# jtdaugherty/flux

Measured on AMD Instinct MI355X. Metric: Msamples/sec on demo2.yml (fixed spp), higher is better.
Workload: dtype f64

## Files before the change

flux_amd/build.py:

```python
import os
import shutil
import subprocess
import sys

ROOT = os.path.dirname(os.path.dirname(os.path.abspath(__file__)))
CSRC = os.path.join(ROOT, "flux_amd", "csrc")
HIP_SOURCES = ["abi.hip", "multi.hip", "tables.hip", "render.hip", "bvh.cpp", "scene_build.cpp", "launch_plan.cpp"]
HIP_HEADERS = ["flux_ctx.h", "scene_build.h", "joining_thread.h", "flux_device.h", "flux_plan.h", "flux_rng.h", "flux_tables.h", "flux_bvh.h", "flux_math.h",
               "flux_math_coeffs.h", "flux_env_verdict.h", "render_body.inc"]
HIP_LIB = os.path.join(ROOT, "flux_amd", "libflux_hip.so")

HIP_FLAGS = ["--offload-arch=gfx950", "-O3", "-std=c++17", "-fPIC", "-shared", "-ffp-contract=off",
             "-fno-fast-math", "-Wall", "-Wno-unused-function",
             "-mllvm", "-disable-machine-licm"]


def _newer(target, deps):
    if not os.path.exists(target):
        return True
    t = os.path.getmtime(target)
    return any(os.path.getmtime(d) > t for d in deps)


def _hipcc():
    for cand in (os.environ.get("HIPCC"), shutil.which("hipcc"), "/opt/rocm/bin/hipcc"):
        if cand and os.path.exists(cand):
            return cand
    raise RuntimeError("hipcc not found (set HIPCC)")


KERNEL_FILES = ["render.hip", "render_body.inc", "tables.hip", "flux_device.h", "flux_plan.h", "flux_bvh.h", "flux_math.h",
                "flux_math_coeffs.h", "flux_rng.h", "flux_tables.h", "flux_env_verdict.h"]


def build_id(extra_flags=()):
    import hashlib

    def digest(names):
        h = hashlib.sha256()
        h.update(" ".join(HIP_FLAGS + list(extra_flags)).encode())
        for n in names:
            path = os.path.join(ROOT, "include", n) if n == "flux_abi.h" else os.path.join(CSRC, n)
            h.update(n.encode() + b"\0")
            with open(path, "rb") as f:
                h.update(f.read())
        return h.hexdigest()[:16]
    return f"lib:{digest(sorted(set(HIP_SOURCES + HIP_HEADERS + ['flux_abi.h'])))} kernels:{digest(KERNEL_FILES)}"


def _id_flag(extra_flags=()):
    return "-DFLUX_BUILD_ID=\"" + build_id(extra_flags) + "\""


def build_variant(out_path, extra_flags, verbose=False):
    srcs = [os.path.join(CSRC, s) for s in HIP_SOURCES]
    flags = [f for f in HIP_FLAGS if not (f == "-ffp-contract=off" and any(x.startswith("-ffp-contract") for x in extra_flags))]
    cmd = [_hipcc()] + flags + list(extra_flags) + [_id_flag(extra_flags), "-o", out_path] + srcs
    if verbose:
        print(" ".join(cmd), file=sys.stderr)
    subprocess.run(cmd, check=True, cwd=CSRC)
    return out_path


def build_hip(force=False, verbose=False):
    srcs = [os.path.join(CSRC, s) for s in HIP_SOURCES]
# ... 38 lines not shown
```

flux_amd/csrc/abi.hip:

```cpp
#include <hip/hip_runtime.h>

#include <chrono>
#include <cmath>
#include <cstdarg>
#include <cstdio>
#include <cstring>
#include <memory>
#include <new>
#include <algorithm>
#include <cstdlib>
#include <string>
#include <vector>

#include "../../include/flux_abi.h"
#include "flux_device.h"
#include "flux_tables.h"
#include "flux_math_coeffs.h"

#include "flux_ctx.h"

namespace flux {

thread_local std::string g_last_error;

// ... 491 lines not shown
    p.first_row = 0;
    p.row_stride = 1;
    p.num_rows = (int32_t)ctx->H;
    p.set_first = (int32_t)first_set;
    p.set_stride = (int32_t)set_stride;
    p.set_count = (int32_t)num_sets;
    p.out_by_set = 1;
    p.slot_first = (int32_t)((first_set - ctx->sets.first) / ctx->sets.stride);
    p.slot_stride = (int32_t)(set_stride / ctx->sets.stride);
    return apply_traversal(ctx, p);
}

int flux_ctx_launch_plan(flux_ctx *ctx, uint64_t num_rows, uint64_t num_sets, int64_t out[FLUX_PLAN_WORDS]) {
    if (!ctx || !out) return fail(FLUX_E_INVALID, "null argument");
    if (num_rows > ctx->H) return fail(FLUX_E_INVALID, "%llu rows exceed image height %u", (unsigned long long)num_rows, ctx->H);
    flux::RenderParams p;
    if (num_sets == 0) {
        p = rows_params(ctx, 0, 1, num_rows, nullptr);
    } else {
        const uint64_t held = ctx->sets.count;
        if (num_sets > held) return fail(FLUX_E_INVALID, "%llu sets exceed the %llu this context holds", (unsigned long long)num_sets,
                                         (unsigned long long)held);
        p = sets_params(ctx, ctx->sets.first, ctx->sets.stride, num_sets, nullptr);
    }
    const flux::LaunchPlan L = flux::plan_render(p, ctx->variant, effective_math(ctx));
    out[0] = L.kernel;
    out[1] = L.block;
    out[2] = (int64_t)L.blocks;
    out[3] = (int64_t)L.lds;
    out[4] = L.waves_per_pixel;
    out[5] = effective_math(ctx);
    out[6] = (ctx->math == FLUX_MATH_FAST && ctx->rp.glossy_long) ? (strict_fits_lds(ctx) ? FLUX_ROUTE_TO_STRICT : FLUX_ROUTE_KEPT_FAST)
                                                                 : FLUX_ROUTE_NONE;
    out[7] = 0;
    return FLUX_OK;
}

int flux_render_rows_device(flux_ctx *ctx, uint64_t first_row, uint64_t row_stride, uint64_t num_rows,
                            void *d_out_rgb, void *hip_stream) {
    if (!ctx) return fail(FLUX_E_INVALID, "null context");
    if (num_rows == 0) return FLUX_OK;
    if (!d_out_rgb) return fail(FLUX_E_INVALID, "null output pointer");
    if (row_stride < 1) return fail(FLUX_E_INVALID, "row_stride must be >= 1");
    if (!holds_all_sets(ctx))
        return fail(FLUX_E_INVALID, "rendering rows needs all sample sets; this context holds the share %u + k*%u "
                    "(flux_ctx_create_sets): use flux_render_sets_device", ctx->sets.first, ctx->sets.stride);
    if (first_row >= ctx->H || first_row + (num_rows - 1) * row_stride >= ctx->H)
        return fail(FLUX_E_INVALID, "rows %llu + k*%llu (k<%llu) exceed image height %u",
                    (unsigned long long)first_row, (unsigned long long)row_stride,
                    (unsigned long long)num_rows, ctx->H);
    DeviceGuard guard(ctx->device);
    if (!guard.ok) return fail(FLUX_E_DEVICE, "hipSetDevice(%d) failed", ctx->device);
    hipStream_t stream = (hipStream_t)hip_stream;
    const flux::RenderParams p = rows_params(ctx, first_row, row_stride, num_rows, (double *)d_out_rgb);
    if (int rc = check_lds_budget(ctx, p, "flux_render_rows")) return rc;
    HIP_TRY(hipEventRecord(ctx->ev0, stream));
    HIP_TRY(flux::launch_render(p, ctx->variant, effective_math(ctx), stream));
    HIP_TRY(hipEventRecord(ctx->ev1, stream));
    ctx->timed = true;
    return FLUX_OK;
}

int flux_render_sets_device(flux_ctx *ctx, uint64_t first_set, uint64_t set_stride, uint64_t num_sets, void *d_out_rgb,
                            void *hip_stream) {
    if (!ctx) return fail(FLUX_E_INVALID, "null context");
    if (num_sets == 0) return FLUX_OK;
    if (!d_out_rgb) return fail(FLUX_E_INVALID, "null output pointer");
// ... 205 lines not shown
```

flux_amd/csrc/flux_device.h:

```cpp
#pragma once
#include <hip/hip_runtime.h>
#include <stdint.h>

#include "flux_bvh.h"
#include "flux_env_verdict.h"


#ifndef FLUX_UNI_SPHERES
#define FLUX_UNI_SPHERES 2
#endif
#ifndef FLUX_BVH_WIDE_MAX_STACK
#define FLUX_BVH_WIDE_MAX_STACK 48
#endif
#ifndef FLUX_MAX_WAVES_PER_PIXEL
#define FLUX_MAX_WAVES_PER_PIXEL 4
#endif
#ifndef FLUX_MIN_SAMPLES_PER_WAVE
#define FLUX_MIN_SAMPLES_PER_WAVE 4096
#endif

namespace flux {

constexpr int kHemiDoubles = 4;
constexpr double kTMin = 0.0005;
constexpr double kPi = 3.14159265358979323846264338327950288;
constexpr double kInvPi = 1.0 / kPi;

constexpr int kShapeSphere = 0;
constexpr int kShapePlane = 1;
constexpr int kShapeDisk = 2;
constexpr int kShapeBox = 3;
constexpr int kMatMatte = 0;
constexpr int kMatEmissive = 1;
constexpr int kMatReflective = 2;
constexpr int kMatGlossy = 3;
constexpr int kMatDielectric = 4;

struct DevShape {
// ... 157 lines not shown
```

flux_amd/csrc/flux_plan.h:

```cpp
#pragma once
#include <stddef.h>
#include <stdint.h>

#include "flux_device.h"

#ifndef FLUX_BLOCK_THREADS
#define FLUX_BLOCK_THREADS 64
#endif
#ifndef FLUX_WPE_SPLIT
#define FLUX_WPE_SPLIT 5
#endif
#ifndef FLUX_HITQ_MIN_TAKE
#define FLUX_HITQ_MIN_TAKE 32
#endif

namespace flux {

constexpr int kGlossExpSlots = 4;

constexpr int kQueueDoubles = 9;
constexpr int kQueueBytesPerWave = (kQueueDoubles * 64) * 8 + 2 * 64 * 4;
constexpr int kHitQDoubles = 7;
constexpr int kHitQInts = 3;
constexpr int kHitQBytesPerSlot = kHitQDoubles * 8 + kHitQInts * 4;
enum HitQField : uint32_t {
    kHitQOx = 0, kHitQOy = 2, kHitQOz = 4, kHitQDx = 6, kHitQDy = 8, kHitQDz = 10, kHitQT = 12,
    kHitQHitDepth = 14,
    kHitQSample = 15,
    kHitQList = 16,
};
constexpr uint32_t kHitQDwordsPerSlot = kHitQBytesPerSlot / 4;
constexpr uint32_t hitq_entry_dword(uint32_t C, uint32_t k) { return (C - 1u - k) * kHitQDwordsPerSlot; }
constexpr bool hitq_admits_phase_a(uint32_t C, uint32_t nhit) { return nhit + 64u <= C; }

constexpr size_t kTputEntryBytes = 24;
constexpr size_t kTputTableMaxBytes = (size_t)4 << 20;
constexpr uint32_t tput_index(uint32_t list_bits, uint32_t ml) { return (1u << list_bits) | ml; }
size_t tput_table_bytes(const RenderParams &p, int *bits = nullptr);

enum KernelCopy { kCopyStrict = 0, kCopyFast = 1, kCopyFastDiel = 2 };
KernelCopy kernel_copy(const RenderParams &p, int math);

struct LaunchPlan {
    int kernel = -1;
    unsigned block = 64;
    uint64_t blocks = 0;
    size_t lds = 0;
    unsigned waves_per_pixel = 1;
    int lds_scene = 0;
    int hq_cap = 0, hq_th = 0, hq_bits = 0;
    int copy = kCopyFast;
    int tris = 0;
    int typ = 0;
    int max32 = 0;
    int uniform_a = 1;
};
LaunchPlan plan_render(const RenderParams &p, int variant, int math);

size_t lane_stacks_lds(int math, size_t depth, bool tris, size_t bvh_stack, size_t lanes);
size_t shade_rays_lds(const RenderParams &p, int math);

}
```

flux_amd/csrc/launch_plan.cpp:

```cpp
#include <algorithm>
#include <cstdlib>

#include "flux_plan.h"
#include "../../include/flux_abi.h"

namespace flux {

KernelCopy kernel_copy(const RenderParams &p, int math) {
    if (math == FLUX_MATH_STRICT) return kCopyStrict;
    return p.has_diel ? kCopyFastDiel : kCopyFast;
}

size_t lane_stacks_lds(int math, size_t depth, bool tris, size_t bvh_stack, size_t lanes) {
    return (math == FLUX_MATH_STRICT ? depth * 4 * lanes * sizeof(double) : 0) + (tris ? bvh_stack * lanes * sizeof(int) : 0);
}

size_t shade_rays_lds(const RenderParams &p, int math) {
    return lane_stacks_lds(math, (size_t)p.max_depth, p.n_tris > 0, (size_t)p.bvh_stack, 64);
}

static bool split_typ(const RenderParams &p) {
    return p.n_sph <= 32 && p.glossy_long == 0 && p.unit_dirs == 1 && p.self_skip == 1 && p.env_short == 1 && p.n_uni == 1 &&
           p.fsph32 != nullptr && p.n_dsk == 0 && p.n_box == 0 && p.has_diel == 0 && (p.n_gloss_exp == 0 || p.gx_stride != 0);
}
// ... 65 lines not shown
        L.block = 64;
        size_t lds4 = (size_t)(p.bvh4_stack > 0 ? p.bvh4_stack : 1) * 64 * sizeof(int);
        const size_t scene4 = (size_t)hit_records(p) * sizeof(DevHitRec) + (size_t)p.n_mats * sizeof(DevMaterial) +
                              (size_t)p.n_sph * sizeof(DevScanSphere);
        const bool lds_scene4 = lds4 + scene4 <= 7680;
        if (lds_scene4) lds4 += scene4;
        if (p.nodes4 != nullptr && p.bvh4_stack <= FLUX_BVH_WIDE_MAX_STACK) {
            L.kernel = 4;
            L.lds = lds4;
            L.lds_scene = lds_scene4 ? 1 : 0;
            L.typ = bvh4_typ(p, lds_scene4) ? 1 : 0;
        } else {
            L.kernel = 3;
            L.lds = (size_t)p.bvh_stack * 64 * sizeof(int);
        }
        return L;
    }
    const size_t scene_lds = split_scene_lds(p);
    if (fast && variant == FLUX_KERNEL_SPLIT && split_serves(p)) {
        L.kernel = 2;
        L.block = block;
        L.waves_per_pixel = K;
        L.lds = (size_t)kQueueBytesPerWave * K + scene_lds;
        L.typ = split_typ(p) ? 1 : 0;
        L.max32 = p.n_sph <= 32 ? 1 : 0;
        if (const char *e = std::getenv("FLUX_SPLIT_UNIFORM_A")) L.uniform_a = std::atoi(e) != 0 ? 1 : 0;
        uint32_t cap, th;
        int bits;
        if (plan_hitq(p, K, scene_lds, cap, th, bits)) {
            L.hq_cap = (int)cap;
            L.hq_th = (int)th;
            L.hq_bits = bits;
            L.lds = (size_t)cap * kHitQBytesPerSlot * K + scene_lds;
        }
        return L;
    }
    L.kernel = variant == FLUX_KERNEL_STATIC ? 0 : 1;
    L.block = block;
    L.waves_per_pixel = variant == FLUX_KERNEL_STATIC ? 1 : K;
    L.lds = lane_stacks_lds(math, (size_t)p.max_depth, tris, (size_t)p.bvh_stack, block);
    L.tris = tris ? 1 : 0;
    return L;
}

}
```

flux_amd/csrc/render_body.inc:

```

#undef FLUX_STAGE
#if FLUX_FAST
#define FLUX_STAGE() __builtin_amdgcn_sched_barrier(0)
#else
#define FLUX_STAGE() ((void)0)
#endif

struct Ray {
    double ox, oy, oz, dx, dy, dz;
};

typedef const __attribute__((address_space(4))) RenderParams *ParamsInKernarg;
static_assert(sizeof(DevMaterial) % 16 == 0, "the bounce-weight records behind the materials are read as double2");
__device__ __forceinline__ const RenderParams &relaunder_params(uint32_t tick) {
    ParamsInKernarg p = (ParamsInKernarg)__builtin_amdgcn_kernarg_segment_ptr();
    asm("" : "+s"(p) : "s"(tick));
    return *(const RenderParams *)p;
}

__device__ __forceinline__ unsigned long long ballot64(bool b) { return __builtin_amdgcn_ballot_w64(b); }
__device__ __forceinline__ bool any64(bool b) { return __builtin_amdgcn_ballot_w64(b) != 0ull; }
__device__ __forceinline__ bool all64(bool b) { return __builtin_amdgcn_ballot_w64(!b) == 0ull; }

typedef double flux_d2 __attribute__((ext_vector_type(2)));
// ... 377 lines not shown
            best = P.n_sph + P.n_pln + j;
            best_id = S.id;
            tb = t;
        }
    }
}

__device__ __forceinline__ void scan_boxes(const RenderParams &P, const Ray &r, double tmin, int &best, int &best_id, double &tb) {
    if (P.n_box <= 0) return;
    const BoxRay A = box_ray(r);
    const int rec0 = P.n_sph + P.n_pln + P.n_dsk;
    for (int j = 0; j < P.n_box; ++j) {
        const DevScanBox &S = P.fbox[j];
        double t;
        int face;
        if (box_shape_hit(S.c0x, S.c0y, S.c0z, S.c1x, S.c1y, S.c1z, r, A, tmin, t, face) &&
            (best < 0 || t < tb || (t == tb && S.id < best_id))) {
            best = rec0 + 6 * j + face;
            best_id = S.id;
            tb = t;
        }
    }
}

constexpr int kFaceDqHi = 0x3d719799;
constexpr float kFaceEnvFront = 1.8446744073709552e19f;
__device__ __forceinline__ float sphere_facing(double dq, bool near_root) {
    const float hq = __int_as_float(__double2hiint(dq));
    return near_root ? -hq : hq;
}
__device__ __forceinline__ bool facing_known(int facing) { return (facing & 0x7fffffff) > kFaceDqHi; }
__device__ __forceinline__ bool facing_front(int facing, int inv_rad_hi) { return (facing ^ inv_rad_hi) < 0; }

template <bool ENV_SHORT = false, bool LDS_SCENE = false, bool MAX32 = false, bool TYP = false, int ZF = -1, bool FACING = false>
__device__ __forceinline__ void scan_shapes_fast(const RenderParams &P, const Ray &r, int self, int &best, double &tb,
                                                 long long *lap = nullptr, const char *fsph_lds = nullptr, int *facing = nullptr) {
    (void)fsph_lds;
    (void)facing;
    constexpr bool FACE = FACING && ZF == 0;
    float face = 0.0f;
    int best_id = -1;
    const double tmin = P.t_min;
    int j0 = 0;
    if (P.n_pln > 0) {
        const DevScanPlane &S = P.fpln[0];
        const double num = (S.px - r.ox) * S.nx + (S.py - r.oy) * S.ny + (S.pz - r.oz) * S.nz;
        const double den = r.dx * S.nx + r.dy * S.ny + r.dz * S.nz;
        const double t = num / den;
        const bool take = t > tmin;
        best = take ? P.n_sph : -1;
        best_id = S.id;
        tb = (ENV_SHORT || take) ? t : tb;
        j0 = 1;
    }
    for (int j = j0; j < P.n_pln; ++j) {
        const DevScanPlane &S = P.fpln[j];
        const double num = (S.px - r.ox) * S.nx + (S.py - r.oy) * S.ny + (S.pz - r.oz) * S.nz;
        const double den = r.dx * S.nx + r.dy * S.ny + r.dz * S.nz;
        const double t = num / den;
        if (t > tmin && (best < 0 || t < tb)) {
            best = P.n_sph + j;
            best_id = S.id;
            tb = t;
        }
    }
    if (!TYP) {
        scan_disks(P, r, tmin, best, best_id, tb);
        scan_boxes(P, r, tmin, best, best_id, tb);
    }
    const bool p_unit_dirs = TYP ? true : P.unit_dirs != 0;
    const bool p_env_short = TYP ? true : P.env_short != 0;
// ... 23 lines not shown
        const int lim = MAX32 ? P.n_sph : ((P.n_sph - base) < 32 ? (P.n_sph - base) : 32);
        uint32_t cand = 0;
        if (f32_filter) {
            cand = MAX32 ? sphere_filter32_laid_out(P, F32) : sphere_filter32(P, F32, base, lim);
            const uint32_t valid_bits = MAX32 ? P.f32_valid : (lim == 32 ? 0xffffffffu : (1u << lim) - 1u);
            cand = big ? valid_bits : (cand & valid_bits);
            const uint32_t sb = (uint32_t)(self - base);
            cand &= ~(sb < 32u ? 1u << sb : 0u);
        } else
        {
#pragma unroll 4
        for (int k = 0; k < lim; ++k) {
            const DevScanSphere S = P.fsph[base + k];
            const double tx = r.ox - S.px, ty = r.oy - S.py, tz = r.oz - S.pz;
            const double hb = sphere_hb(tx, ty, tz, ux, uy, uz);
            const double c = __builtin_fma(tx, tx, __builtin_fma(ty, ty, __builtin_fma(tz, tz, -S.rr)));
            const double dq = __builtin_fma(hb, hb, -c);
            const int hq = __double2hiint(dq);
            const int hc = __double2hiint(c);
            const int hmin = min(hc, __double2hiint(hb));
            if (hq >= 0 && hmin <= 0) cand |= 1u << k;
        }
        }
        if (any_zflat) {
            if (zflat)
                for (uint32_t m = cand; m;) {
                    const int k = __builtin_ctz(m);
                    m &= m - 1;
                    if (box_z_nan_miss(P, r, base + k)) cand &= ~(1u << k);
                }
        }
        lap_stamp(lap, 3);
        uint32_t todo = cand;
        if (todo) {
            auto record = [&](int k) {
                if constexpr (LDS_SCENE)
                    return *reinterpret_cast<const DevScanSphere *>(fsph_lds + (uint32_t)(base + k) * (uint32_t)sizeof(DevScanSphere));
                else
                    return *reinterpret_cast<const DevScanSphere *>(
                        reinterpret_cast<const char *>(P.fsph) + (uint32_t)(base + k) * (uint32_t)sizeof(DevScanSphere));
            };
            int k = __builtin_ctz(todo);
            todo &= todo - 1;
            DevScanSphere Sk = record(k);
            for (;;) {
                FLUX_TRIP(P, 11);
                FLUX_CENSUS(P, 4);
                const double tx = r.ox - Sk.px, ty = r.oy - Sk.py, tz = r.oz - Sk.pz;
                const double hb = sphere_hb(tx, ty, tz, ux, uy, uz);
                const double c = __builtin_fma(tx, tx, __builtin_fma(ty, ty, __builtin_fma(tz, tz, -Sk.rr)));
                const double dq = __builtin_fma(hb, hb, -c);
                if (dq >= 0.0) {
                    const double e = fastmath::fsqrt_nonneg(dq);
                    double t = (-hb - e) * rs;
                    const float face_k = sphere_facing(dq, t > tmin);
                    if (!(t > tmin)) t = (-hb + e) * rs;
                    if (t > tmin) {
                        bool take = best < 0 || t < tb;
                        if (!take && t == tb && best >= P.n_sph) take = P.frec[base + k].orig_id < best_id;
                        if (take) {
                            best = base + k;
                            tb = t;
                            if (FACE) face = face_k;
                        }
                    }
                }
                if (!todo) break;
                k = __builtin_ctz(todo);
                todo &= todo - 1;
                Sk = record(k);
            }
        }
        lap_stamp(lap, 4);
    }
    if (f32_filter) {
        for (int j = 0; j < p_n_uni; ++j) {
            FLUX_CENSUS(P, 5);
            const int k = P.uni_idx[j];
            if (ENV32 && p_env_short && p_unit_dirs) {
                float g_lo, g_hi;
                env_g32(E32, (float)tb, g_lo, g_hi);
                if ((ballot64(!(E32.cp < P.env32.deep)) | (ballot64(best >= 0) & ballot64(!(g_lo > 0.0f)) & ballot64(!(g_hi < 0.0f)))) == 0ull) {
                    if (best < 0 || g_lo > 0.0f) {
                        best = k;
                        tb = 2.0 * P.env_radius;
                        if (FACE) face = kFaceEnvFront;
                    }
                    continue;
                }
            }
            const DevScanSphere S = TYP ? DevScanSphere{P.env_px, P.env_py, P.env_pz, P.env_rr} : P.fsph[k];
            const double tx = r.ox - S.px, ty = r.oy - S.py, tz = r.oz - S.pz;
            const double hb = sphere_hb(tx, ty, tz, ux, uy, uz);
            const double c = __builtin_fma(tx, tx, __builtin_fma(ty, ty, __builtin_fma(tz, tz, -S.rr)));
            const double dq = __builtin_fma(hb, hb, -c);
            if (ENV_SHORT && p_env_short && p_unit_dirs && !any_zflat) {
                const bool deep = c < P.env_deep;
// ... 472 lines not shown
    const V3 d = mk(p.r.dx, p.r.dy, p.r.dz);
    const V3 pt = mk(p.r.ox + t * d.x, p.r.oy + t * d.y, p.r.oz + t * d.z);
    V3 n = mk(0.0, 0.0, 1.0);
    int kind = kMatEmissive;
    bool unit_n = true;
    bool convex = false;
    double fr = 0.0, fg = 0.0, fb = 0.0, m_inv_e1 = 0.0, ax = 0.0, az = 0.0;
    if (hit < 0) {
        Lr = P.bgr;
        Lg = P.bgg;
        Lb = P.bgb;
        if (STATS) st.c[6]++;
    } else {
        if (is_tri) {
            const DevTri &T = P.tris[slot];
            const DevMaterial &Mt = P.mats[T.mat];
            p.mat = T.mat;
            n = mk(T.nx, T.ny, T.nz);
            kind = Mt.kind;
            fr = Mt.fr; fg = Mt.fg; fb = Mt.fb; m_inv_e1 = Mt.inv_e1;
            ax = kind == kMatMatte ? 0.0034 : 0.00424;
            az = kind == kMatMatte ? 0.0071 : 0.00764;
        } else {
            p.mat = analytic_hit_fields<LDS_SCENE, UNI>(P, p.r, hit, t, frec_lds, n, kind, unit_n, convex, fr, fg, fb, m_inv_e1, ax, az);
        }
        if (kind == kMatEmissive) {
            if (STATS) st.c[5]++;
            bool front;
            if (FACING && ballot64(!facing_known(facing)) == 0ull) {
                const DevHitRec &R = *reinterpret_cast<const DevHitRec *>(frec_lds + (uint32_t)hit * (uint32_t)sizeof(DevHitRec));
                front = facing_front(facing, reinterpret_cast<const int *>(&R.inv_rad)[1]);
            } else {
                front = ((n.x * -1.0) * d.x + (n.y * -1.0) * d.y + (n.z * -1.0) * d.z) > 0.0;
            }
            Lr = fr;
            Lg = fg;
            Lb = fb;
            if (ballot64(!front) != 0ull) {
                Lr = front ? fr : 0.0;
                Lg = front ? fg : 0.0;
                Lb = front ? fb : 0.0;
            }
        } else {
            if (UNI) {
                if (BOUNCE) fast_bounce<STATS, TRIS, TYP, FIRST, true>(P, p, set, i, hit, slot, t, n, d, pt, kind, fr, fg, fb, m_inv_e1, ax, az,
                                                                       unit_n, convex, is_tri, st, cz);
                return true;
            }
            bounce = 1;
        }
    }
    if (UNI) return false;
    asm("" : "+v"(bounce));
    if (BOUNCE && bounce) {
        fast_bounce<STATS, TRIS, TYP, FIRST>(P, p, set, i, hit, slot, t, n, d, pt, kind, fr, fg, fb, m_inv_e1, ax, az, unit_n, convex, is_tri, st,
                                            cz);
    }
    return bounce != 0;
}

template <bool STATS, bool TYP>
__device__ __forceinline__ void bounce_parked_hit(const RenderParams &P, Path &p, uint32_t set, uint32_t i, int hit, double t, Stats &st,
                                                  int cz, const char *frec_lds) {
    const V3 d = mk(p.r.dx, p.r.dy, p.r.dz);
    const V3 pt = mk(p.r.ox + t * d.x, p.r.oy + t * d.y, p.r.oz + t * d.z);
    V3 n;
// ... 595 lines not shown
                if (take) {
                    best = k;
                    tb = t;
                }
            }
        }
    }
}

__device__ __forceinline__ double lds_dword_pair(const uint32_t *p) { return __hiloint2double((int)p[1], (int)p[0]); }
__device__ __forceinline__ void lds_dword_pair_store(uint32_t *p, double v) {
    p[0] = (uint32_t)__double2loint(v);
    p[1] = (uint32_t)__double2hiint(v);
}

__device__ __forceinline__ uint32_t *hitq_entry(uint32_t *pool, uint32_t C, uint32_t k) {
    return reinterpret_cast<uint32_t *>(reinterpret_cast<char *>(pool) + __umul24(C - 1u - k, (uint32_t)kHitQBytesPerSlot));
}

template <bool STATS, bool TYP, bool UNIFORM_A>
__device__ __forceinline__ bool shade_primary_hits(const RenderParams &P, Path &p, uint32_t set, uint32_t ia, int hit, double t, double &Lr,
                                                   double &Lg, double &Lb, Stats &st, const char *frec_lds, int uni_a) {
    if (UNIFORM_A) {
        const int hu = __builtin_amdgcn_readfirstlane(hit);
        if (uni_a != 0 && ballot64(hit != hu) == 0ull) {
            FLUX_CENSUS(P, 16);
            return shade_hit_fast<STATS, false, true, TYP, true, true, false, true>(P, p, set, ia, hu, -1, t, Lr, Lg, Lb, st, 3, frec_lds);
        }
    }
    FLUX_CENSUS(P, 17);
    return shade_hit_fast<STATS, false, true, TYP, true>(P, p, set, ia, hit, -1, t, Lr, Lg, Lb, st, 3, frec_lds);
}
constexpr bool split_uniform_a(bool TYP, bool HQ) { return HQ || TYP; }

template <bool STATS, bool MAX32, bool TYP, bool HQ = false>
__global__ __launch_bounds__(64 * FLUX_MAX_WAVES_PER_PIXEL, FLUX_WPE_SPLIT) void render_split_kernel(const RenderParams P0, int hq_cap, int hq_th,
                                                                                                  int hq_bits, int uni_a) {
    (void)hq_cap;
    (void)hq_th;
    (void)hq_bits;
    const RenderParams &P = P0;
    extern __shared__ double lds_stack[];
    __shared__ double part[FLUX_MAX_WAVES_PER_PIXEL][3];
    const int tid = threadIdx.x;
    const uint32_t lane = tid & 63;
    const uint32_t N = P.nsamp;
    const uint32_t K = blockDim.x >> 6, sub = (uint32_t)__builtin_amdgcn_readfirstlane(tid >> 6);
    const uint32_t s_lo = (uint32_t)((uint64_t)N * sub / K), s_hi = (uint32_t)((uint64_t)N * (sub + 1) / K);
    const int n_rec = TYP ? P.n_sph + P.n_pln + P.n_dsk : hit_records(P);
    const size_t scene_lds_bytes = (size_t)n_rec * sizeof(DevHitRec) + (size_t)P.n_sph * sizeof(DevScanSphere);
    double *q = lds_stack + scene_lds_bytes / 8 + (size_t)sub * (HQ ? (size_t)hq_cap * kHitQBytesPerSlot / 8 : kQueueBytesPerWave / 8);
    int *qi = reinterpret_cast<int *>(q + (size_t)kQueueDoubles * 64);
    const char *const frec_lds = reinterpret_cast<const char *>(lds_stack);
    const char *const fsph_lds = frec_lds + (size_t)n_rec * sizeof(DevHitRec);
    {
        uint32_t *dst = reinterpret_cast<uint32_t *>(const_cast<char *>(frec_lds));
        const uint32_t nrec_w = (uint32_t)n_rec * (uint32_t)(sizeof(DevHitRec) / 4), nsph_w = (uint32_t)P.n_sph * 8u;
        const uint32_t *src_r = reinterpret_cast<const uint32_t *>(P.frec), *src_s = reinterpret_cast<const uint32_t *>(P.fsph);
        for (uint32_t w = (uint32_t)tid; w < nrec_w; w += blockDim.x) dst[w] = src_r[w];
        for (uint32_t w = (uint32_t)tid; w < nsph_w; w += blockDim.x) dst[nrec_w + w] = src_s[w];
        __syncthreads();
    }
    const uint64_t wave = blockIdx.x;
    int lrow = 0, col = 0, row = 0;
    uint32_t set = 0;
    uint64_t pixel = 0;
    const bool wave_on = map_wave(P, wave, lrow, col, row, set, pixel);
    set = (uint32_t)__builtin_amdgcn_readfirstlane((int)set);
    col = __builtin_amdgcn_readfirstlane(col);
    row = __builtin_amdgcn_readfirstlane(row);
// ... 56 lines not shown
                    cont = shade_primary_hits<STATS, TYP, split_uniform_a(TYP, HQ)>(P, p, set_p, ia, hit, t, Lr, Lg, Lb, st, frec_lds, uni_a);
                    if (cont && p.depth > P.max_depth) {
                        cont = false;
                        Lr = Lg = Lb = 0.0;
                        if (STATS) st.c[7]++;
                    }
                    if (!cont) {
                        fold_path(p, nullptr, 0, Lr, Lg, Lb);
                        sr += Lr;
                        sg += Lg;
                        sb += Lb;
                    }
                }
                i = ia;
                ml = (uint32_t)hit;
                if (!cont) p.depth = kDeadDepth;
            }
            if (nhit) {
                const unsigned long long freemask = ballot64(p.depth == kDeadDepth);
                const uint32_t nfree = (uint32_t)__popcll(freemask);
                const uint32_t take = nfree < nhit ? nfree : nhit;
                if (!run_a || take >= H || !(next < s_hi && hitq_admits_phase_a(C, nhit))) {
                    const uint32_t rank = __builtin_amdgcn_mbcnt_hi((uint32_t)(freemask >> 32),
                                                                    __builtin_amdgcn_mbcnt_lo((uint32_t)freemask, 0u));
                    if (p.depth == kDeadDepth && rank < take) {
                        FLUX_CENSUS(P, 15);
                        const uint32_t *e = hitq_entry(pool, C, nhit - 1u - rank);
                        p.r.ox = lds_dword_pair(e + kHitQOx);
                        p.r.oy = lds_dword_pair(e + kHitQOy);
                        p.r.oz = lds_dword_pair(e + kHitQOz);
                        p.r.dx = lds_dword_pair(e + kHitQDx);
                        p.r.dy = lds_dword_pair(e + kHitQDy);
                        p.r.dz = lds_dword_pair(e + kHitQDz);
                        const double t = lds_dword_pair(e + kHitQT);
                        const int hd = (int)e[kHitQHitDepth];
                        i = e[kHitQSample];
                        const int hit = hd & 0xffff;
                        p.depth = hd >> 16;
                        ml = e[kHitQList];
                        const uint32_t list_bits = __umul24((uint32_t)(p.depth - 1), (uint32_t)hq_bits);
                        if (P.tput != nullptr) {
                            const uint32_t off = __umul24(tput_index(list_bits, ml), (uint32_t)kTputEntryBytes);
                            p.tr = gather_global<double>(P.tput, off);
                            p.tg = gather_global<double>(P.tput, off + 8u);
                            p.tb = gather_global<double>(P.tput, off + 16u);
                        } else {
                            const DevHitRec &R0 = recs[ml & bmask];
                            p.tr = R0.fr;
                            p.tg = R0.fg;
                            p.tb = R0.fb;
#pragma unroll 1
                            for (int k = 1; k < p.depth - 1; ++k) {
                                const DevHitRec &Rk = recs[(ml >> (k * hq_bits)) & bmask];
                                p.tr *= Rk.fr;
                                p.tg *= Rk.fg;
                                p.tb *= Rk.fb;
                            }
                        }
                        ml |= (uint32_t)hit << list_bits;
                        bounce_parked_hit<STATS, TYP>(P, p, set_p, i, hit, t, st, 6, frec_lds);
                    }
                    nhit -= take;
                }
            }
            if (__builtin_expect((nhit | (s_hi - next)) == 0u, 0)) {
                if (!any64(p.depth != kDeadDepth)) break;
            }
            FLUX_TRIP(P, 10);
            const bool live = p.depth != kDeadDepth;
            const bool trace = p.depth <= P.max_depth;
            double Lr = 0.0, Lg = 0.0, Lb = 0.0;
            bool cont = false;
            int hit = -1;
            double t = 0.0;
            if (trace) {
                FLUX_CENSUS(P, 3);
                if (STATS) st.c[1]++;
                const float ofx = (float)p.r.ox, ofy = (float)p.r.oy, ofz = (float)p.r.oz;
                const float oo32 = __builtin_fmaf(ofz, ofz, __builtin_fmaf(ofy, ofy, ofx * ofx));
                int facing;
                if (__builtin_expect((ballot64(p.r.dz == 0.0) | ballot64(!(oo32 < 0.999e6f))) != 0ull, 0))
                    scan_shapes_fast<true, true, MAX32, TYP, 1, true>(P, p.r, p.self, hit, t, nullptr, fsph_lds, &facing);
                else
                    scan_shapes_fast<true, true, MAX32, TYP, 0, true>(P, p.r, p.self, hit, t, nullptr, fsph_lds, &facing);
                cont = shade_hit_fast<STATS, false, true, TYP, false, false, true>(P, p, set_p, i, hit, -1, t, Lr, Lg, Lb, st, 0, frec_lds, facing);
            }
            if (live && !cont) {
                if (STATS && !trace) st.c[7]++;
                fold_path(p, nullptr, 0, Lr, Lg, Lb);
                sr += Lr;
                sg += Lg;
                sb += Lb;
            }
            const unsigned long long pmask = ballot64(cont);
            if (cont) {
                uint32_t *e = hitq_entry(pool, C, nhit + __builtin_amdgcn_mbcnt_hi((uint32_t)(pmask >> 32),
                                                                                   __builtin_amdgcn_mbcnt_lo((uint32_t)pmask, 0u)));
                lds_dword_pair_store(e + kHitQOx, p.r.ox);
                lds_dword_pair_store(e + kHitQOy, p.r.oy);
                lds_dword_pair_store(e + kHitQOz, p.r.oz);
                lds_dword_pair_store(e + kHitQDx, p.r.dx);
                lds_dword_pair_store(e + kHitQDy, p.r.dy);
                lds_dword_pair_store(e + kHitQDz, p.r.dz);
                lds_dword_pair_store(e + kHitQT, t);
                e[kHitQHitDepth] = (uint32_t)(hit | (p.depth << 16));
                e[kHitQSample] = i;
                e[kHitQList] = ml;
            }
            nhit += (uint32_t)__popcll(pmask);
        }
    }
    if (!HQ && wave_on) {
        unsigned long long cand_mask, in_mask;
        double in_t0;
        pixel_sphere_mask(P, row, col, lane, cand_mask, in_mask, in_t0);

#ifdef FLUX_DEBUG_CLOCK
        long long lap_store[8] = {0, 0, 0, 0, 0, 0, 0, (long long)__builtin_readcyclecounter()};
        long long *lap = lap_store;
#else
        long long *lap = nullptr;
#endif
        uint32_t next = s_lo;
        uint32_t qcount = 0;
        uint32_t i = 0;
        constexpr int kDeadDepth = 0x7fffffff;
        Path p;
        path_begin(p);
        p.depth = kDeadDepth;
        p.sq = make_double2(0.0, 0.0);
        p.r = Ray{0, 0, 0, 0, 0, 1};
        for (;;) {
            const RenderParams &P = relaunder_params(next + qcount);
            uint32_t set_p = set;
            unsigned long long cand_p = cand_mask, in_p = in_mask;
            asm("" : "+s"(set_p) : "s"(next));
            asm("" : "+s"(cand_p), "+s"(in_p) : "s"(next));
            auto pop = [&]() {
// ... 809 lines not shown
#define FLUX_LAUNCH(K)                                                     \
    do {                                                                   \
        if (stats && tris) K<true, true><<<g, b, lds, stream>>>(p);        \
        else if (stats) K<true, false><<<g, b, lds, stream>>>(p);          \
        else if (tris) K<false, true><<<g, b, lds, stream>>>(p);           \
        else K<false, false><<<g, b, lds, stream>>>(p);                    \
    } while (0)
#if FLUX_FAST
    if (L.kernel == 3) {
        if (stats) render_bvh_kernel<true><<<g, b, lds, stream>>>(p);
        else render_bvh_kernel<false><<<g, b, lds, stream>>>(p);
        return hipGetLastError();
    }
    if (L.kernel == 4) {
        if (L.typ) {
#if FLUX_DIEL
            return hipErrorInvalidValue;
#else
            if (stats) render_bvh4_kernel<true, true, true><<<g, b, lds, stream>>>(p);
            else render_bvh4_kernel<false, true, true><<<g, b, lds, stream>>>(p);
#endif
        } else if (L.lds_scene) {
            if (stats) render_bvh4_kernel<true, true, false><<<g, b, lds, stream>>>(p);
            else render_bvh4_kernel<false, true, false><<<g, b, lds, stream>>>(p);
        } else {
            if (stats) render_bvh4_kernel<true, false, false><<<g, b, lds, stream>>>(p);
            else render_bvh4_kernel<false, false, false><<<g, b, lds, stream>>>(p);
        }
        return hipGetLastError();
    }
    if (L.kernel == 2) {
        const int c = L.hq_cap, h = L.hq_th, bits = L.hq_bits;
        const bool hq = L.hq_cap > 0;
        RenderParams ps = p;
        if (!hq || ps.tput_bits != bits) ps.tput = nullptr;
#define FLUX_LAUNCH_SPLIT(MAX32, TYP, HQ)                                                                      \
    do {                                                                                                       \
        if (stats) render_split_kernel<true, MAX32, TYP, HQ><<<g, b, lds, stream>>>(ps, c, h, bits, L.uniform_a);  \
        else render_split_kernel<false, MAX32, TYP, HQ><<<g, b, lds, stream>>>(ps, c, h, bits, L.uniform_a);   \
    } while (0)
#if FLUX_DIEL
        if (L.typ || hq) return hipErrorInvalidValue;
#else
        if (L.typ) {
            if (hq) FLUX_LAUNCH_SPLIT(true, true, true);
            else FLUX_LAUNCH_SPLIT(true, true, false);
            return hipGetLastError();
        }
        if (hq) {
            if (L.max32) FLUX_LAUNCH_SPLIT(true, false, true);
            else FLUX_LAUNCH_SPLIT(false, false, true);
            return hipGetLastError();
        }
#endif
        if (L.max32) FLUX_LAUNCH_SPLIT(true, false, false);
        else FLUX_LAUNCH_SPLIT(false, false, false);
#undef FLUX_LAUNCH_SPLIT
        return hipGetLastError();
    }
#endif
    if (L.kernel == 0)
        FLUX_LAUNCH(render_static_kernel);
    else
        FLUX_LAUNCH(render_refill_kernel);
#undef FLUX_LAUNCH
    return hipGetLastError();
}
```

flux_amd/render.py:

```python
import ctypes as C

import numpy as np

from . import _lib
from .scene import JobConfiguration, SceneData, SceneDesc, WorkUnit, WorkUnitResult

STAT_NAMES = ("samples", "segments", "matte_bounces", "glossy_bounces", "specular_bounces",
              "emissive_hits", "misses", "depth_exhausted", "bvh_nodes", "tris_tested",
              "dielectric_reflections", "dielectric_transmissions")


class Renderer:
    def __init__(self, scene_data: SceneData, config: JobConfiguration, seed: int = 1, device: int = 0,
                 set_share=None):
        self.scene_data = scene_data
        self.config = config
        self.seed = int(seed)
        self.device = int(device)
        self.width = scene_data.output_settings.image_width
        self.height = scene_data.output_settings.image_height
        self._desc = SceneDesc(scene_data)
        cfg = _lib.FluxJobCfg(config.sample_root, config.max_trace_depth, config.rows_per_work_unit)
        h = C.c_void_p()
        self.set_share = (0, 1) if set_share is None else (int(set_share[0]), int(set_share[1]))
# ... 106 lines not shown
        _lib.check(_lib.lib.flux_ctx_set_math(self._handle(), mode))
        self.requested_math = int(mode)
        self._warn_if_routed()

    def last_kernel_ms(self) -> float:
        return float(_lib.lib.flux_ctx_last_kernel_ms(self._handle()))

    def enable_stats(self, on=True):
        _lib.check(_lib.lib.flux_ctx_enable_stats(self._handle(), 1 if on else 0))

    def stats(self, reset=False) -> dict:
        buf = (C.c_uint64 * _lib.NUM_STATS)()
        _lib.check(_lib.lib.flux_ctx_stats(self._handle(), buf, 1 if reset else 0))
        return dict(zip(STAT_NAMES, [int(x) for x in buf]))

    def stats_raw(self) -> list:
        buf = (C.c_uint64 * _lib.NUM_STATS)()
        _lib.check(_lib.lib.flux_ctx_stats(self._handle(), buf, 0))
        return [int(x) for x in buf]

    def set_traversal(self, mode: int):
        _lib.check(_lib.lib.flux_ctx_set_traversal(self._handle(), mode))

    def bvh_info(self) -> dict:
        buf = (C.c_uint64 * _lib.BVH_INFO_WORDS)()
        _lib.check(_lib.lib.flux_ctx_bvh_info(self._handle(), buf, _lib.BVH_INFO_WORDS))
        names = ("nodes", "triangles", "max_depth", "max_leaf", "node_bytes", "tri_bytes", "build_us", "wide_nodes",
                 "leaf_records", "fused_leaves", "wide_stack", "wide_node_bytes", "leaf_record_bytes", "wide_in_use")
        return dict(zip(names, [int(x) for x in buf]))

    def launch_plan(self, num_rows=None, num_sets: int = 0) -> dict:
        buf = (C.c_int64 * _lib.PLAN_WORDS)()
        _lib.check(_lib.lib.flux_ctx_launch_plan(self._handle(), self.height if num_rows is None else num_rows, num_sets, buf))
        names = ("kernel", "block", "blocks", "lds", "waves_per_pixel", "math", "route")
        return dict(zip(names, [int(x) for x in buf]))

    def table(self, which: int) -> np.ndarray:
        S = len(range(self.set_share[0], self.width, self.set_share[1]))
        N = self.config.sample_root ** 2
        D = self.config.max_trace_depth
        shape = (S, N, 2) if which in (_lib.TABLE_PIXEL, _lib.TABLE_DISC) else (S, D, N, 3)
        out = np.empty(shape, dtype=np.float64)
        _lib.check(_lib.lib.flux_ctx_copy_table(self._handle(), which, out.ctypes.data_as(C.POINTER(C.c_double)),
                                                out.size))
        return out

    def row_perm(self, row: int) -> np.ndarray:
        out = np.empty(self.width, dtype=np.int32)
        _lib.check(_lib.lib.flux_ctx_copy_row_perm(self._handle(), row, out.ctypes.data_as(C.POINTER(C.c_int32)),
                                                   out.size))
        return out

    def camera_basis(self) -> np.ndarray:
        out = np.empty(9, dtype=np.float64)
        _lib.check(_lib.lib.flux_ctx_camera_basis(self._handle(), out.ctypes.data_as(C.POINTER(C.c_double))))
        return out.reshape(3, 3)

    def device_bytes(self) -> int:
        return int(_lib.lib.flux_ctx_device_bytes(self._handle()))

    def create_timing(self) -> dict:
        return _create_timing(self._handle())


def _create_timing(handle) -> dict:
    buf = (C.c_double * _lib.CREATE_TIMING_WORDS)()
    _lib.check(_lib.lib.flux_ctx_create_timing(handle, buf))
# ... 146 lines not shown
```

Before: 54760.

## Add f32 sphere candidate pre-pass with deferred exact t in split kernel

Adds a float32 conservative sphere-intersection verdict with error margins that runs first in the split kernel's sphere scan, for the MAX32+TYP+HQ variant. When every lane in the wave reaches a certain verdict, it skips the f64 scan and marks the hit t as deferred. The exact f64 t is then recomputed only when the queued hit is consumed. This is meant to cut f64 arithmetic in the hot intersection loop, but it costs an extra wave-wide pass, more ballots and registers, and a fallback to the full f64 scan whenever any lane is undecided.

```diff
diff --git a/flux_amd/build.py b/flux_amd/build.py
--- a/flux_amd/build.py
+++ b/flux_amd/build.py
@@ -7,7 +7,7 @@
 CSRC = os.path.join(ROOT, "flux_amd", "csrc")
 HIP_SOURCES = ["abi.hip", "multi.hip", "tables.hip", "render.hip", "bvh.cpp", "scene_build.cpp", "launch_plan.cpp"]
 HIP_HEADERS = ["flux_ctx.h", "scene_build.h", "joining_thread.h", "flux_device.h", "flux_plan.h", "flux_rng.h", "flux_tables.h", "flux_bvh.h", "flux_math.h",
-               "flux_math_coeffs.h", "flux_env_verdict.h", "render_body.inc"]
+               "flux_math_coeffs.h", "flux_env_verdict.h", "flux_sphere_verdict.h", "render_body.inc"]
 HIP_LIB = os.path.join(ROOT, "flux_amd", "libflux_hip.so")
 
 HIP_FLAGS = ["--offload-arch=gfx950", "-O3", "-std=c++17", "-fPIC", "-shared", "-ffp-contract=off",
@@ -30,7 +30,7 @@
 
 
 KERNEL_FILES = ["render.hip", "render_body.inc", "tables.hip", "flux_device.h", "flux_plan.h", "flux_bvh.h", "flux_math.h",
-                "flux_math_coeffs.h", "flux_rng.h", "flux_tables.h", "flux_env_verdict.h"]
+                "flux_math_coeffs.h", "flux_rng.h", "flux_tables.h", "flux_env_verdict.h", "flux_sphere_verdict.h"]
 
 
 def build_id(extra_flags=()):
diff --git a/flux_amd/csrc/abi.hip b/flux_amd/csrc/abi.hip
--- a/flux_amd/csrc/abi.hip
+++ b/flux_amd/csrc/abi.hip
@@ -547,7 +547,7 @@
     out[5] = effective_math(ctx);
     out[6] = (ctx->math == FLUX_MATH_FAST && ctx->rp.glossy_long) ? (strict_fits_lds(ctx) ? FLUX_ROUTE_TO_STRICT : FLUX_ROUTE_KEPT_FAST)
                                                                  : FLUX_ROUTE_NONE;
-    out[7] = 0;
+    out[7] = L.f32_candidates;
     return FLUX_OK;
 }
 
diff --git a/flux_amd/csrc/flux_device.h b/flux_amd/csrc/flux_device.h
--- a/flux_amd/csrc/flux_device.h
+++ b/flux_amd/csrc/flux_device.h
@@ -4,6 +4,7 @@
 
 #include "flux_bvh.h"
 #include "flux_env_verdict.h"
+#include "flux_sphere_verdict.h"
 
 
 #ifndef FLUX_UNI_SPHERES
diff --git a/flux_amd/csrc/flux_plan.h b/flux_amd/csrc/flux_plan.h
--- a/flux_amd/csrc/flux_plan.h
+++ b/flux_amd/csrc/flux_plan.h
@@ -54,6 +54,7 @@
     int typ = 0;
     int max32 = 0;
     int uniform_a = 1;
+    int f32_candidates = 0;
 };
 LaunchPlan plan_render(const RenderParams &p, int variant, int math);
 
diff --git a/flux_amd/csrc/flux_sphere_verdict.h b/flux_amd/csrc/flux_sphere_verdict.h
--- /dev/null
+++ b/flux_amd/csrc/flux_sphere_verdict.h
@@ -0,0 +1,111 @@
+#pragma once
+#include <cmath>
+
+#if defined(__HIPCC__) || defined(__CUDACC__)
+#define FLUX_SPH_HD __host__ __device__ inline __attribute__((always_inline))
+#else
+#define FLUX_SPH_HD inline
+#endif
+
+namespace flux {
+
+FLUX_SPH_HD double sph_rsq_seed(double x) {
+#if defined(__HIP_DEVICE_COMPILE__)
+    return __builtin_amdgcn_rsq(x);
+#else
+    return 1.0 / std::sqrt(x);
+#endif
+}
+FLUX_SPH_HD double sph_sqrt_nonneg(double x) {
+    const double y0 = sph_rsq_seed(x + 4.9406564584124654e-324);
+    double g = x * y0;
+    double h = 0.5 * y0;
+    const double r = __builtin_fma(-h, g, 0.5);
+    g = __builtin_fma(g, r, g);
+    h = __builtin_fma(h, r, h);
+    const double d = __builtin_fma(-g, g, x);
+    return __builtin_fma(d, h, g);
+}
+FLUX_SPH_HD double sph_hb(double tx, double ty, double tz, double ux, double uy, double uz) {
+    return __builtin_fma(tz, uz, __builtin_fma(ty, uy, tx * ux));
+}
+FLUX_SPH_HD bool sphere_hit_exact(double ox, double oy, double oz, double ux, double uy, double uz, double rs, double px, double py, double pz,
+                                  double rr, double tmin, double &t, double &dq, bool &near_root) {
+    const double tx = ox - px, ty = oy - py, tz = oz - pz;
+    const double hb = sph_hb(tx, ty, tz, ux, uy, uz);
+    const double c = __builtin_fma(tx, tx, __builtin_fma(ty, ty, __builtin_fma(tz, tz, -rr)));
+    dq = __builtin_fma(hb, hb, -c);
+    near_root = false;
+    t = 0.0;
+    if (!(dq >= 0.0)) return false;
+    const double e = sph_sqrt_nonneg(dq);
+    t = (-hb - e) * rs;
+    near_root = t > tmin;
+    if (!near_root) t = (-hb + e) * rs;
+    return t > tmin;
+}
+
+constexpr int kSphUndecided = 0, kSphMiss = 1, kSphHit = 2;
+constexpr float kSphMarginDq = 6e-6f;
+constexpr float kSphMarginT = 1.25f;
+constexpr float kSphFaceFloor = 1.001e-12f;
+constexpr float kSphFaceKnown = 1.8446744073709552e19f;
+
+struct Sphere32 {
+    float px, py, pz, rr;
+};
+FLUX_SPH_HD Sphere32 sphere32(double px, double py, double pz, double rr) { return Sphere32{(float)px, (float)py, (float)pz, (float)rr}; }
+FLUX_SPH_HD void sph_tmin32(double tmin, float &lo, float &hi) {
+    const float f = (float)tmin;
+    lo = f * (1.0f - 1.1920929e-7f);
+    hi = f * (1.0f + 1.1920929e-7f);
+}
+FLUX_SPH_HD float sph_plane_w(float tbf) { return __builtin_fabsf(tbf) * 2.3841858e-7f; }
+
+FLUX_SPH_HD int sphere_verdict32(const Sphere32 &S, float ox, float oy, float oz, float ux, float uy, float uz, float oo, float tmin_lo,
+                                 float tmin_hi, float &t, float &mt, bool &near_root) {
+    const float tx = ox - S.px, ty = oy - S.py, tz = oz - S.pz;
+    const float hb = __builtin_fmaf(tz, uz, __builtin_fmaf(ty, uy, tx * ux));
+    const float tt = __builtin_fmaf(tz, tz, __builtin_fmaf(ty, ty, tx * tx));
+    const float c = tt - S.rr;
+    const float dq = __builtin_fmaf(hb, hb, -c);
+    const float m = kSphMarginDq * ((oo + tt) + S.rr);
+    t = 0.0f;
+    mt = 0.0f;
+    near_root = false;
+    if (dq < -m) return kSphMiss;
+    if (!(dq > m + kSphFaceFloor)) return kSphUndecided;
+#if defined(__HIP_DEVICE_COMPILE__)
+    const float y = __builtin_amdgcn_rsqf(dq);
+#else
+    const float y = 1.0f / std::sqrt(dq);
+#endif
+    const float e = dq * y;
+    mt = (kSphMarginT * m) * y;
+    const float t1 = -hb - e;
+    if (t1 - mt > tmin_hi) {
+        t = t1;
+        near_root = true;
+        return kSphHit;
+    }
+    if (!(t1 + mt < tmin_lo)) return kSphUndecided;
+    const float t2 = e - hb;
+    if (t2 - mt > tmin_hi) {
+        t = t2;
+        return kSphHit;
+    }
+    return t2 + mt < tmin_lo ? kSphMiss : kSphUndecided;
+}
+
+FLUX_SPH_HD int sphere_replace32(bool has_best, float t, float mt, float tb, float w) {
+    if (!has_best) return 1;
+    if (t + mt < tb - w) return 1;
+    if (t - mt > tb + w) return 0;
+    return -1;
+}
+
+FLUX_SPH_HD float env_widen32(float tb, float w, float hb2) {
+    return 1.01f * (w * (__builtin_fmaf(2.0f, __builtin_fabsf(tb), __builtin_fabsf(hb2)) + w));
+}
+
+}
diff --git a/flux_amd/csrc/launch_plan.cpp b/flux_amd/csrc/launch_plan.cpp
--- a/flux_amd/csrc/launch_plan.cpp
+++ b/flux_amd/csrc/launch_plan.cpp
@@ -121,6 +121,8 @@
             L.hq_th = (int)th;
             L.hq_bits = bits;
             L.lds = (size_t)cap * kHitQBytesPerSlot * K + scene_lds;
+            L.f32_candidates = (L.typ && L.max32) ? 1 : 0;
+            if (const char *e = std::getenv("FLUX_SPLIT_F32_CANDIDATES")) L.f32_candidates = (L.f32_candidates && std::atoi(e) != 0) ? 1 : 0;
         }
         return L;
     }
diff --git a/flux_amd/csrc/render_body.inc b/flux_amd/csrc/render_body.inc
--- a/flux_amd/csrc/render_body.inc
+++ b/flux_amd/csrc/render_body.inc
@@ -433,11 +433,17 @@
 __device__ __forceinline__ bool facing_known(int facing) { return (facing & 0x7fffffff) > kFaceDqHi; }
 __device__ __forceinline__ bool facing_front(int facing, int inv_rad_hi) { return (facing ^ inv_rad_hi) < 0; }
 
-template <bool ENV_SHORT = false, bool LDS_SCENE = false, bool MAX32 = false, bool TYP = false, int ZF = -1, bool FACING = false>
+template <bool ENV_SHORT = false, bool LDS_SCENE = false, bool MAX32 = false, bool TYP = false, int ZF = -1, bool FACING = false,
+          bool F32C = false>
 __device__ __forceinline__ void scan_shapes_fast(const RenderParams &P, const Ray &r, int self, int &best, double &tb,
-                                                 long long *lap = nullptr, const char *fsph_lds = nullptr, int *facing = nullptr) {
+                                                 long long *lap = nullptr, const char *fsph_lds = nullptr, int *facing = nullptr,
+                                                 int f32c_on = 0, bool *t_deferred = nullptr) {
     (void)fsph_lds;
     (void)facing;
+    (void)f32c_on;
+    (void)t_deferred;
+    constexpr bool F32C_HERE = F32C && ENV_SHORT && LDS_SCENE && MAX32 && TYP && ZF == 0 && FACING;
+    if (F32C_HERE) *t_deferred = false;
     constexpr bool FACE = FACING && ZF == 0;
     float face = 0.0f;
     int best_id = -1;
@@ -527,37 +533,78 @@
         }
         lap_stamp(lap, 3);
         uint32_t todo = cand;
+        auto record = [&](int k) {
+            if constexpr (LDS_SCENE)
+                return *reinterpret_cast<const DevScanSphere *>(fsph_lds + (uint32_t)(base + k) * (uint32_t)sizeof(DevScanSphere));
+            else
+                return *reinterpret_cast<const DevScanSphere *>(
+                    reinterpret_cast<const char *>(P.fsph) + (uint32_t)(base + k) * (uint32_t)sizeof(DevScanSphere));
+        };
+        if constexpr (F32C_HERE) {
+            if (f32c_on != 0) {
+                const float ofx = (float)r.ox, ofy = (float)r.oy, ofz = (float)r.oz;
+                const float ufx = (float)ux, ufy = (float)uy, ufz = (float)uz;
+                float tlo, thi;
+                sph_tmin32(tmin, tlo, thi);
+                int b32 = best;
+                float tbf = (float)tb, w = sph_plane_w(tbf), face32 = 0.0f;
+                int und = 0;
+                for (uint32_t m = cand; m;) {
+                    const int k = __builtin_ctz(m);
+                    m &= m - 1;
+                    const DevScanSphere Sk = record(k);
+                    float t32, mt;
+                    bool near32;
+                    const int v = sphere_verdict32(sphere32(Sk.px, Sk.py, Sk.pz, Sk.rr), ofx, ofy, ofz, ufx, ufy, ufz, oof, tlo, thi, t32, mt, near32);
+                    und |= (int)(v == kSphUndecided);
+                    if (v == kSphHit) {
+                        const int rep = sphere_replace32(b32 >= 0, t32, mt, tbf, w);
+                        und |= rep >> 1;
+                        if (rep > 0) {
+                            b32 = k;
+                            tbf = t32;
+                            w = mt;
+                            face32 = near32 ? -kSphFaceKnown : kSphFaceKnown;
+                        }
+                    }
+                }
+                float g_lo, g_hi;
+                env_g32(E32, tbf, g_lo, g_hi);
+                const float gw = env_widen32(tbf, w, E32.hb2);
+                g_lo -= gw;
+                g_hi += gw;
+                if ((ballot64(und != 0) | ballot64(!(E32.cp < P.env32.deep)) |
+                     (ballot64(b32 >= 0) & ballot64(!(g_lo > 0.0f)) & ballot64(!(g_hi < 0.0f)))) == 0ull) {
+                    FLUX_CENSUS(P, 18);
+                    const bool env_wins = b32 < 0 || g_lo > 0.0f;
+                    const bool sphere_wins = !env_wins && b32 < P.n_sph;
+                    *t_deferred = sphere_wins;
+                    tb = env_wins ? 2.0 * P.env_radius : (sphere_wins ? (double)tbf : tb);
+                    best = env_wins ? P.uni_idx[0] : b32;
+                    face = env_wins ? kFaceEnvFront : face32;
+                    *facing = __float_as_int(face);
+                    return;
+                }
+                FLUX_CENSUS(P, 19);
+            }
+        }
         if (todo) {
-            auto record = [&](int k) {
-                if constexpr (LDS_SCENE)
-                    return *reinterpret_cast<const DevScanSphere *>(fsph_lds + (uint32_t)(base + k) * (uint32_t)sizeof(DevScanSphere));
-                else
-                    return *reinterpret_cast<const DevScanSphere *>(
-                        reinterpret_cast<const char *>(P.fsph) + (uint32_t)(base + k) * (uint32_t)sizeof(DevScanSphere));
-            };
             int k = __builtin_ctz(todo);
             todo &= todo - 1;
             DevScanSphere Sk = record(k);
             for (;;) {
                 FLUX_TRIP(P, 11);
                 FLUX_CENSUS(P, 4);
-                const double tx = r.ox - Sk.px, ty = r.oy - Sk.py, tz = r.oz - Sk.pz;
-                const double hb = sphere_hb(tx, ty, tz, ux, uy, uz);
-                const double c = __builtin_fma(tx, tx, __builtin_fma(ty, ty, __builtin_fma(tz, tz, -Sk.rr)));
-                const double dq = __builtin_fma(hb, hb, -c);
-                if (dq >= 0.0) {
-                    const double e = fastmath::fsqrt_nonneg(dq);
-                    double t = (-hb - e) * rs;
-                    const float face_k = sphere_facing(dq, t > tmin);
-                    if (!(t > tmin)) t = (-hb + e) * rs;
-                    if (t > tmin) {
-                        bool take = best < 0 || t < tb;
-                        if (!take && t == tb && best >= P.n_sph) take = P.frec[base + k].orig_id < best_id;
-                        if (take) {
-                            best = base + k;
-                            tb = t;
-                            if (FACE) face = face_k;
-                        }
+                double t, dq;
+                bool near_k;
+                if (sphere_hit_exact(r.ox, r.oy, r.oz, ux, uy, uz, rs, Sk.px, Sk.py, Sk.pz, Sk.rr, tmin, t, dq, near_k)) {
+                    const float face_k = sphere_facing(dq, near_k);
+                    bool take = best < 0 || t < tb;
+                    if (!take && t == tb && best >= P.n_sph) take = P.frec[base + k].orig_id < best_id;
+                    if (take) {
+                        best = base + k;
+                        tb = t;
+                        if (FACE) face = face_k;
                     }
                 }
                 if (!todo) break;
@@ -1096,6 +1143,10 @@
                 front = facing_front(facing, reinterpret_cast<const int *>(&R.inv_rad)[1]);
             } else {
                 front = ((n.x * -1.0) * d.x + (n.y * -1.0) * d.y + (n.z * -1.0) * d.z) > 0.0;
+                if (FACING) {
+                    const DevHitRec &R = *reinterpret_cast<const DevHitRec *>(frec_lds + (uint32_t)(hit < 0 ? 0 : hit) * (uint32_t)sizeof(DevHitRec));
+                    if (facing_known(facing)) front = facing_front(facing, reinterpret_cast<const int *>(&R.inv_rad)[1]);
+                }
             }
             Lr = fr;
             Lg = fg;
@@ -1757,10 +1808,14 @@
     return shade_hit_fast<STATS, false, true, TYP, true>(P, p, set, ia, hit, -1, t, Lr, Lg, Lb, st, 3, frec_lds);
 }
 constexpr bool split_uniform_a(bool TYP, bool HQ) { return HQ || TYP; }
+constexpr bool split_f32_candidates(bool MAX32, bool TYP, bool HQ) { return MAX32 && TYP && HQ; }
+constexpr int kHitQTDeferred = 0x8000, kHitQHitMask = 0x7fff;
 
 template <bool STATS, bool MAX32, bool TYP, bool HQ = false>
 __global__ __launch_bounds__(64 * FLUX_MAX_WAVES_PER_PIXEL, FLUX_WPE_SPLIT) void render_split_kernel(const RenderParams P0, int hq_cap, int hq_th,
-                                                                                                  int hq_bits, int uni_a) {
+                                                                                                  int hq_bits, int launch_flags) {
+    const int uni_a = launch_flags & 1, f32c = launch_flags & 2;
+    (void)f32c;
     (void)hq_cap;
     (void)hq_th;
     (void)hq_bits;
@@ -1883,11 +1938,21 @@
                         p.r.dx = lds_dword_pair(e + kHitQDx);
                         p.r.dy = lds_dword_pair(e + kHitQDy);
                         p.r.dz = lds_dword_pair(e + kHitQDz);
-                        const double t = lds_dword_pair(e + kHitQT);
+                        double t = lds_dword_pair(e + kHitQT);
                         const int hd = (int)e[kHitQHitDepth];
                         i = e[kHitQSample];
-                        const int hit = hd & 0xffff;
+                        const int hit = hd & (split_f32_candidates(MAX32, TYP, HQ) ? kHitQHitMask : 0xffff);
                         p.depth = hd >> 16;
+                        if (split_f32_candidates(MAX32, TYP, HQ)) {
+                            if (ballot64((hd & kHitQTDeferred) != 0) != 0ull) {
+                                if ((hd & kHitQTDeferred) != 0) {
+                                    const DevScanSphere Sk = *reinterpret_cast<const DevScanSphere *>(fsph_lds + (uint32_t)hit * (uint32_t)sizeof(DevScanSphere));
+                                    double dq;
+                                    bool near_k;
+                                    sphere_hit_exact(p.r.ox, p.r.oy, p.r.oz, p.r.dx, p.r.dy, p.r.dz, 1.0, Sk.px, Sk.py, Sk.pz, Sk.rr, P.t_min, t, dq, near_k);
+                                }
+                            }
+                        }
                         ml = e[kHitQList];
                         const uint32_t list_bits = __umul24((uint32_t)(p.depth - 1), (uint32_t)hq_bits);
                         if (P.tput != nullptr) {
@@ -1924,6 +1989,7 @@
             bool cont = false;
             int hit = -1;
             double t = 0.0;
+            bool t_deferred = false;
             if (trace) {
                 FLUX_CENSUS(P, 3);
                 if (STATS) st.c[1]++;
@@ -1933,7 +1999,8 @@
                 if (__builtin_expect((ballot64(p.r.dz == 0.0) | ballot64(!(oo32 < 0.999e6f))) != 0ull, 0))
                     scan_shapes_fast<true, true, MAX32, TYP, 1, true>(P, p.r, p.self, hit, t, nullptr, fsph_lds, &facing);
                 else
-                    scan_shapes_fast<true, true, MAX32, TYP, 0, true>(P, p.r, p.self, hit, t, nullptr, fsph_lds, &facing);
+                    scan_shapes_fast<true, true, MAX32, TYP, 0, true, split_f32_candidates(MAX32, TYP, HQ)>(P, p.r, p.self, hit, t, nullptr, fsph_lds,
+                                                                                                            &facing, f32c, &t_deferred);
                 cont = shade_hit_fast<STATS, false, true, TYP, false, false, true>(P, p, set_p, i, hit, -1, t, Lr, Lg, Lb, st, 0, frec_lds, facing);
             }
             if (live && !cont) {
@@ -1954,7 +2021,7 @@
                 lds_dword_pair_store(e + kHitQDy, p.r.dy);
                 lds_dword_pair_store(e + kHitQDz, p.r.dz);
                 lds_dword_pair_store(e + kHitQT, t);
-                e[kHitQHitDepth] = (uint32_t)(hit | (p.depth << 16));
+                e[kHitQHitDepth] = (uint32_t)(hit | (split_f32_candidates(MAX32, TYP, HQ) && t_deferred ? kHitQTDeferred : 0) | (p.depth << 16));
                 e[kHitQSample] = i;
                 e[kHitQList] = ml;
             }
@@ -2830,12 +2897,13 @@
     if (L.kernel == 2) {
         const int c = L.hq_cap, h = L.hq_th, bits = L.hq_bits;
         const bool hq = L.hq_cap > 0;
+        const int flags = (L.uniform_a ? 1 : 0) | (L.f32_candidates ? 2 : 0);
         RenderParams ps = p;
         if (!hq || ps.tput_bits != bits) ps.tput = nullptr;
 #define FLUX_LAUNCH_SPLIT(MAX32, TYP, HQ)                                                                      \
     do {                                                                                                       \
-        if (stats) render_split_kernel<true, MAX32, TYP, HQ><<<g, b, lds, stream>>>(ps, c, h, bits, L.uniform_a);  \
-        else render_split_kernel<false, MAX32, TYP, HQ><<<g, b, lds, stream>>>(ps, c, h, bits, L.uniform_a);   \
+        if (stats) render_split_kernel<true, MAX32, TYP, HQ><<<g, b, lds, stream>>>(ps, c, h, bits, flags);  \
+        else render_split_kernel<false, MAX32, TYP, HQ><<<g, b, lds, stream>>>(ps, c, h, bits, flags);   \
     } while (0)
 #if FLUX_DIEL
         if (L.typ || hq) return hipErrorInvalidValue;
diff --git a/flux_amd/render.py b/flux_amd/render.py
--- a/flux_amd/render.py
+++ b/flux_amd/render.py
@@ -162,7 +162,7 @@
     def launch_plan(self, num_rows=None, num_sets: int = 0) -> dict:
         buf = (C.c_int64 * _lib.PLAN_WORDS)()
         _lib.check(_lib.lib.flux_ctx_launch_plan(self._handle(), self.height if num_rows is None else num_rows, num_sets, buf))
-        names = ("kernel", "block", "blocks", "lds", "waves_per_pixel", "math", "route")
+        names = ("kernel", "block", "blocks", "lds", "waves_per_pixel", "math", "route", "f32_candidates")
         return dict(zip(names, [int(x) for x in buf]))
 
     def table(self, which: int) -> np.ndarray:
```

Result: slower. 51530 (-5.9%).
